# Paleogenomics/pss-bam

Measured on NVIDIA B200. Metric: aligned reads/s (PSS tally), higher is better.
Workload: dtype u64

## Files before the change

### pss-bam_b200/csrc/pss_kernels.cuh

```cuda
#pragma once

#include <cuda_runtime.h>
#include <stdint.h>

#include "pss_record.h"

namespace pssgpu {

__device__ __forceinline__ uint32_t smem_u32(const void *p) { return (uint32_t)__cvta_generic_to_shared(p); }

__device__ __forceinline__ void mbar_init(uint64_t *bar, uint32_t count)
{
    asm volatile("mbarrier.init.shared::cta.b64 [%0], %1;" ::"r"(smem_u32(bar)), "r"(count));
}
__device__ __forceinline__ void fence_mbar_init()
{
    asm volatile("fence.mbarrier_init.release.cluster;" ::: "memory");
}
__device__ __forceinline__ void fence_proxy_async()
{
    asm volatile("fence.proxy.async.shared::cta;" ::: "memory");
}
__device__ __forceinline__ void mbar_expect_tx(uint64_t *bar, uint32_t bytes)
{
// ... 385 lines not shown
        atomicAdd(&s_bins[v.x & 0xffffu], 1u); atomicAdd(&s_bins[v.x >> 16], 1u);
        atomicAdd(&s_bins[v.y & 0xffffu], 1u); atomicAdd(&s_bins[v.y >> 16], 1u);
        atomicAdd(&s_bins[v.z & 0xffffu], 1u); atomicAdd(&s_bins[v.z >> 16], 1u);
        atomicAdd(&s_bins[v.w & 0xffffu], 1u); atomicAdd(&s_bins[v.w >> 16], 1u);
    }
    for (unsigned long long i = a + body * 8 + threadIdx.x; i < hi; i += kSpecSmemThreads) atomicAdd(&s_bins[payload[i]], 1u);
    __syncthreads();
    for (uint32_t i = threadIdx.x; i < (uint32_t)kSpecSmemBins; i += kSpecSmemThreads) {
        const uint32_t v = s_bins[i];
        if (v) atomicAdd(counts + ((size_t)b << kSpecSmemLog) + i, (CT)v);
    }
}
__global__ void __launch_bounds__(256) widen_kernel(const unsigned int *__restrict__ in, unsigned long long *__restrict__ out, uint64_t n)
{
    for (uint64_t i = (uint64_t)blockIdx.x * blockDim.x + threadIdx.x; i < n; i += (uint64_t)gridDim.x * blockDim.x) out[i] = in[i];
}

#ifndef PSS_TALLY_CTAS_PER_SM
#define PSS_TALLY_CTAS_PER_SM 2
#endif
#ifndef PSS_TALLY_THREADS
#define PSS_TALLY_THREADS 256
#endif
#ifndef PSS_TALLY_ITERS
#define PSS_TALLY_ITERS 4
#endif
#ifndef PSS_TALLY_PREFETCH
#define PSS_TALLY_PREFETCH 1
#endif
constexpr int kThreads    = PSS_TALLY_THREADS;
constexpr int kWarps      = kThreads / 32;
#ifndef PSS_TALLY_SLOTS
#define PSS_TALLY_SLOTS (PSS_TALLY_ITERS * PSS_TALLY_THREADS)
#endif
constexpr int kSlots      = PSS_TALLY_SLOTS;
constexpr int kIters      = (kSlots + kThreads - 1) / kThreads;
constexpr int kChunks     = 2 * kSlots;
constexpr int kSpan       = kChunks * 32;
constexpr int kPrefix     = 16;
constexpr int kStageMax   = kSpan - 80;
constexpr int kSegs       = kIters * kWarps;
constexpr int kCacheContigs = 64;
constexpr int kCacheNames   = 1024;
constexpr int kCacheSlots   = 1024;
constexpr int kFlushEvery   = 1900;
static_assert(kThreads % 32 == 0 && kSlots % 32 == 0 && kSegs <= 64, "the newline ranking keeps at most two segment counts per lane");
static_assert(kThreads >= kCacheContigs, "one thread per cached contig fills the shared-memory table");
static_assert(kSpan < (1 << 20) && kThreads <= 1024, "pass A packs a newline position into 20 bits and its rank into the rest");

struct ContigCache {
    uint32_t n;
    uint32_t seed;
    uint16_t name_w0[kCacheContigs], name_len[kCacheContigs];
    uint64_t base_off[kCacheContigs], len[kCacheContigs];
    uint8_t  slot[kCacheSlots];
    uint32_t names32[kCacheNames / 4 + 2 * kCacheContigs];
};

struct TallyShared {
    uint32_t table[2 * 32 * 16];
    uint32_t stats[8];
    uint32_t stats_fk[8];
    ContigCache cc;
};

struct TallySmem {
    alignas(128) uint8_t bytes[kSpan + 32];
    alignas(8) uint32_t le[kChunks + 8];
    uint32_t seg[64];
    uint32_t nlpos[kThreads + 4];
    uint32_t warp_sum[kWarps];
    uint32_t ctl[2];
    unsigned long long long_end;
    TallyShared sh;
    alignas(8) uint64_t bar;
};

struct TallyArgs {
    const uint8_t *sam;
    uint64_t       len;
    const unsigned long long *len_dev;
    uint64_t       stream_off;
    uint64_t       range_bytes;
    unsigned int  *range_ctr;
    uint32_t       one;
    DevGenome      g;
    TallyCfg       cfg;
    TallyCfg       cfg_fk;
    uint32_t       names_bytes;
    uint32_t       cc_seed;
    uint32_t       cc_ok;
    unsigned long long *pss_tables;
    unsigned long long *fk_hist;
    unsigned long long *stats;
    unsigned long long *stats_fk;
    uint64_t           *dbg_off;
    int8_t             *dbg_code;
    unsigned long long *dbg_n;
    uint64_t            dbg_cap;
};

struct SmemAt {
    static constexpr int kLookBack = kPrefix;
    const uint8_t *p;
    __device__ __forceinline__ int lo() const { return 0; }
    __device__ __forceinline__ uint32_t operator()(int i) const { return p[i]; }
    __device__ __forceinline__ uint32_t word(int i) const { return *reinterpret_cast<const uint32_t *>(p + i); }
};
struct SmemRel {
    static constexpr int kLookBack = kPrefix;
    const uint8_t *p;
    __device__ __forceinline__ int lo() const { return -kPrefix; }
    __device__ __forceinline__ uint32_t operator()(int i) const { return p[i]; }
    __device__ __forceinline__ uint32_t word(int i) const
    {
        return (uint32_t)p[i] | ((uint32_t)p[i + 1] << 8) | ((uint32_t)p[i + 2] << 16) | ((uint32_t)p[i + 3] << 24);
    }
};
struct GlobalAt {
    static constexpr int kLookBack = 0;
    const uint8_t *p;
    __device__ __forceinline__ int lo() const { return 0; }
    __device__ __forceinline__ uint32_t operator()(int i) const { return __ldg(p + i); }
    __device__ __forceinline__ uint32_t word(int i) const
    {
        return (uint32_t)__ldg(p + i) | ((uint32_t)__ldg(p + i + 1) << 8) | ((uint32_t)__ldg(p + i + 2) << 16) |
               ((uint32_t)__ldg(p + i + 3) << 24);
    }
};

template <int LUT>
__device__ __forceinline__ uint32_t lop3(uint32_t a, uint32_t b, uint32_t c)
{
    uint32_t d;
    asm("lop3.b32 %0, %1, %2, %3, %4;" : "=r"(d) : "r"(a), "r"(b), "r"(c), "n"(LUT));
    return d;
}
__device__ __forceinline__ uint32_t imad(uint32_t a, uint32_t b, uint32_t c)
{
    uint32_t d;
    asm("mad.lo.u32 %0, %1, %2, %3;" : "=r"(d) : "r"(a), "r"(b), "r"(c));
    return d;
}
__device__ __forceinline__ void classify4(uint32_t w, uint32_t one, uint32_t &zle, uint32_t &znl)
{
    const uint32_t v = w & 0x7f7f7f7fu;
    const uint32_t ge21 = imad(v, one, 0x5f5f5f5fu);
    const uint32_t ge0a = imad(v, one, 0x76767676u);
    const uint32_t ge0b = imad(v, one, 0x75757575u);
    zle = lop3<0x02>(ge21, w, 0x80808080u);
    znl = lop3<0x20>(zle, ge0b, ge0a);
}
__device__ __forceinline__ void classify4_fast(uint32_t w, uint32_t one, uint32_t &zle, uint32_t &p1)
{
    const uint32_t v = w & 0x7f7f7f7fu;
    const uint32_t ge21 = imad(v, one, 0x5f5f5f5fu);
    zle = lop3<0x02>(ge21, w, 0x80808080u);
    p1 = w & 0x02020202u;
}
__device__ __forceinline__ uint32_t gather8(uint32_t z0, uint32_t z1)
{
    return __dp4a(z1, 0x80402010u, __dp4a(z0, 0x08040201u, 0u));
}
__device__ __forceinline__ void classify32(const uint8_t *p, uint32_t one, uint32_t &le32, uint32_t &nl32)
{
    const uint4 v0 = *reinterpret_cast<const uint4 *>(p);
    const uint4 v1 = *reinterpret_cast<const uint4 *>(p + 16);
    uint32_t zl[8], zn[8];
    classify4(v0.x, one, zl[0], zn[0]); classify4(v0.y, one, zl[1], zn[1]);
    classify4(v0.z, one, zl[2], zn[2]); classify4(v0.w, one, zl[3], zn[3]);
    classify4(v1.x, one, zl[4], zn[4]); classify4(v1.y, one, zl[5], zn[5]);
    classify4(v1.z, one, zl[6], zn[6]); classify4(v1.w, one, zl[7], zn[7]);
    le32 = (gather8(zl[0], zl[1]) >> 7) + gather8(zl[2], zl[3]) * 2u + gather8(zl[4], zl[5]) * 512u + gather8(zl[6], zl[7]) * 131072u;
    nl32 = (gather8(zn[0], zn[1]) >> 7) + gather8(zn[2], zn[3]) * 2u + gather8(zn[4], zn[5]) * 512u + gather8(zn[6], zn[7]) * 131072u;
}

__device__ __forceinline__ void classify32_fast(const uint4 &v0, const uint4 &v1, uint32_t one, uint32_t &le32, uint32_t &nc32)
{
    uint32_t zl[8], zp[8];
    classify4_fast(v0.x, one, zl[0], zp[0]); classify4_fast(v0.y, one, zl[1], zp[1]);
    classify4_fast(v0.z, one, zl[2], zp[2]); classify4_fast(v0.w, one, zl[3], zp[3]);
    classify4_fast(v1.x, one, zl[4], zp[4]); classify4_fast(v1.y, one, zl[5], zp[5]);
    classify4_fast(v1.z, one, zl[6], zp[6]); classify4_fast(v1.w, one, zl[7], zp[7]);
    le32 = (gather8(zl[0], zl[1]) >> 7) + gather8(zl[2], zl[3]) * 2u + gather8(zl[4], zl[5]) * 512u + gather8(zl[6], zl[7]) * 131072u;
// ... 372 lines not shown
        r.flag = 0; r.pos = 0; r.mapq = 0; r.tlen = 0;
        r.rname_off = r.cigar_off = r.seq_off = kPrefix; r.rname_len = r.cigar_len = r.seq_len = 0;
    }
    uint64_t   cb, cl;
    const int  ci = lookup_contig(T.cc, A.g, at, r.rname_off, valid ? r.rname_len : 0, cb, cl);
    PssStreams st;
    int        code_fk = code;
    if (MODE != kModePss) {
        FkHits          h;
        const TallyCfg &F = (MODE == kModeBoth) ? A.cfg_fk : A.cfg;
        const int       rc = fk_record(at, r, valid, ci, cb, cl, A.g, F, h);
        if (valid) code_fk = rc;
        if (h.add5) atomicAdd(A.fk_hist + h.idx5, 1ull);
        if (h.add3) atomicAdd(A.fk_hist + (1ull << (2 * F.K)) + h.idx3, 1ull);
    }
    if (MODE != kModeFragkon && NACC == 0) {
        if (valid)
            code = pss_record_wide(at, r, ci, cb, cl, A.g, A.cfg, [&](int tb, int row, int cell) {
                atomicAdd(A.pss_tables + ((size_t)tb * rows + row) * 16 + cell, 1ull);
            });
    } else if (MODE != kModeFragkon) {
        const int rc = pss_record<SmemAt, (ROWS ? ROWS - 2 : -1)>(at, r, valid, ci, cb, cl, A.g, A.cfg, st);
        if (valid) code = rc;
    } else {
        code = code_fk;
    }
    if (code != 99) log_outcome(A, goff, code);
    __syncwarp();
    if (MODE != kModeFragkon && NACC > 0) {
        tally_rows<NACC, ROWS>(st, acc, rows, lane, A.one);
        if (++acc_iters >= kFlushEvery) { flush_acc<NACC>(acc, rows, lane, T.table); acc_iters = 0; }
    }
    {
        const uint32_t m_any = __ballot_sync(full, code != 99);
        const uint32_t m0 = __ballot_sync(full, code == kCounted);
        const uint32_t m1 = __ballot_sync(full, code == kNoContig);
        const uint32_t m2 = __ballot_sync(full, code == kFiltered);
        const uint32_t m3 = __ballot_sync(full, code == kParseFail);
        const uint32_t m4 = __ballot_sync(full, code == kUndefined);
        const uint32_t mine = lane == 0 ? m_any : lane == 1 ? m0 : lane == 2 ? m1 : lane == 3 ? m2 : lane == 4 ? m3 : m4;
        st_acc += (uint32_t)__popc(mine);
        if (MODE == kModeBoth) {
            const uint32_t f0 = __ballot_sync(full, code_fk == kCounted);
            const uint32_t f1 = __ballot_sync(full, code_fk == kNoContig);
            const uint32_t f2 = __ballot_sync(full, code_fk == kFiltered);
            const uint32_t f3 = __ballot_sync(full, code_fk == kParseFail);
            const uint32_t f4 = __ballot_sync(full, code_fk == kUndefined);
            const uint32_t mine_fk = lane == 0 ? m_any : lane == 1 ? f0 : lane == 2 ? f1 : lane == 3 ? f2 : lane == 4 ? f3 : f4;
            st_acc_fk += (uint32_t)__popc(mine_fk);
        }
    }
}

template <int MODE, int NACC, int ROWS>
__global__ void __launch_bounds__(kThreads, PSS_TALLY_CTAS_PER_SM) tally_kernel(const __grid_constant__ TallyArgs A)
{
    extern __shared__ __align__(128) unsigned char smem_raw[];
    TallySmem &S = *reinterpret_cast<TallySmem *>(smem_raw);
    const uint32_t tid = threadIdx.x, lane = tid & 31u, warp = tid >> 5;
    const uint32_t full = 0xffffffffu;
    const uint32_t lt_mask = (1u << lane) - 1u;

    for (uint32_t i = tid; i < 8; i += kThreads) S.le[kChunks + i] = ~0u;
    if (tid < kPrefix) S.bytes[tid] = 'x';
    if (tid == 0) { mbar_init(&S.bar, 1); fence_mbar_init(); }
    cta_prologue(S.sh, A, tid, kThreads);

    const int      rows = A.cfg.R + 2;
    const uint32_t one = A.one;
    uint32_t       phase = 0;
    uint32_t       acc[NACC ? NACC : 1];
    int            acc_iters = 0;
    uint32_t       st_acc = 0, st_acc_fk = 0;
#pragma unroll
    for (int i = 0; i < (NACC ? NACC : 1); i++) acc[i] = 0;
    const uint64_t text_len = A.len_dev ? (uint64_t)__ldg(A.len_dev) : A.len;
    const uint64_t len16 = (text_len + 15) & ~15ull;
    int            est = kStageMax;

    for (;;) {
        __syncthreads();
        if (tid == 0) S.ctl[0] = atomicAdd(A.range_ctr, 1u);
        __syncthreads();
        const uint64_t range_begin = (uint64_t)S.ctl[0] * A.range_bytes;
        if (range_begin >= text_len) break;
        const uint64_t range_end = (range_begin + A.range_bytes < text_len) ? range_begin + A.range_bytes : text_len;
        uint64_t       pos = range_begin;
        bool           want_full = false;

        while (pos < range_end) {
            const uint64_t gsrc = pos ? ((pos - 1) & ~15ull) : 0;
            const int64_t  gbase = (int64_t)gsrc - kPrefix;
            const int      head = (int)((int64_t)pos - 1 - gbase);
            int            want = want_full ? kStageMax : est;
            want = (want + 16) & ~63; want -= 16;
            if (want > kStageMax) want = kStageMax;
            const uint64_t left = len16 - gsrc;
            const bool     sees_end = left <= (uint64_t)want;
            const int      nb = sees_end ? (int)left : want;
            const bool     is_full = sees_end || want >= kStageMax;
            const int      data_end = sees_end ? (int)((int64_t)text_len - gbase) : kPrefix + nb;
            if (tid == 0) {
                fence_proxy_async();
                mbar_expect_tx(&S.bar, (uint32_t)nb);
                bulk_g2s(S.bytes + kPrefix, A.sam + gsrc, (uint32_t)nb, &S.bar);
            }
            if (warp == 0) mbar_wait(&S.bar, phase);
            __syncthreads();
            if (warp != 0) mbar_wait(&S.bar, phase);
            phase ^= 1u;

            const int tail_slot = data_end >> 6;
            const int n_valid = 2 * (sees_end ? tail_slot + 1 : tail_slot);
            if (tid == 0) {
                S.bytes[kPrefix - 1] = pos == 0 ? '\n' : 'x';
                for (int i = kPrefix; i < head; i++) S.bytes[i] = 'x';
            }
            if (sees_end && tid == (uint32_t)(tail_slot % kThreads)) {
                S.bytes[data_end] = '\n';
                for (int i = data_end + 1; i < 64 * (tail_slot + 1); i++) S.bytes[i] = 'x';
            }

            constexpr uint32_t kNoNl = 0xfffffu;
            uint32_t pk[kIters];
            uint32_t redo = 0;
            const uint32_t r4 = (lane >> 1) & 3u;
            const uint32_t qo0 = 16u * r4, qo1 = 16u * (1u ^ r4), qo2 = 16u * (2u ^ r4), qo3 = 16u * (3u ^ r4);
            const uint32_t rot16 = 16u * (r4 & 1u), hi_x = r4 >> 1, swz = 16u * r4;
#pragma unroll
            for (int it = 0; it < kIters; it++) {
                pk[it] = kNoNl;
                if (it * 2 * kThreads < n_valid + 8 && ((it + 1) * kThreads <= kSlots || it * kThreads + (int)tid < kSlots)) {
                    const int      c = 2 * (it * kThreads + (int)tid);
                    const uint8_t *src = S.bytes + 32 * c;
                    const uint4    q0 = *reinterpret_cast<const uint4 *>(src + qo0), q1 = *reinterpret_cast<const uint4 *>(src + qo1);
                    const uint4    q2 = *reinterpret_cast<const uint4 *>(src + qo2), q3 = *reinterpret_cast<const uint4 *>(src + qo3);
                    uint32_t le_x, nc_x, le_y, nc_y;
                    classify32_fast(q0, q1, one, le_x, nc_x);
                    classify32_fast(q2, q3, one, le_y, nc_y);
                    le_x = __funnelshift_l(le_x, le_x, rot16);
                    le_y = __funnelshift_l(le_y, le_y, rot16);
                    S.le[c + (int)hi_x] = le_x;
                    S.le[c + 1 - (int)hi_x] = le_y;
                    const bool     has = (nc_x | nc_y) != 0u && c < n_valid;
                    const uint32_t b = __ballot_sync(full, has);
                    const uint32_t rank = (uint32_t)__popc(b & lt_mask);
                    const uint32_t x = nc_x ? nc_x : nc_y;
                    const uint32_t p = (uint32_t)(32 * c) + ((((nc_x ? 0u : 32u) + (uint32_t)__ffs((int)x) - 1u) ^ swz) & 63u);
                    redo |= has ? ((x & (x - 1u)) | (nc_x ? nc_y : 0u) | ((uint32_t)S.bytes[has ? p : 0u] ^ 0x0au)) : 0u;
                    pk[it] = has ? (p + (rank << 20)) : kNoNl;
                    if (lane == 0) S.seg[it * kWarps + (int)warp] = b;
                } else if (lane == 0) {
                    S.seg[it * kWarps + (int)warp] = 0u;
                }
            }
            const int any_multi = __syncthreads_or((int)(redo != 0u));
            if (tid < 8) S.le[n_valid + (int)tid] = ~0u;

            uint32_t n_nl;
            if (!any_multi) {
                uint32_t v0 = (lane < (uint32_t)kSegs) ? (uint32_t)__popc(S.seg[lane]) : 0u;
                uint32_t v1 = (kSegs > 32 && lane + 32 < (uint32_t)kSegs) ? (uint32_t)__popc(S.seg[lane + 32]) : 0u;
                uint32_t x = v0 | (v1 << 16);
                uint32_t inc = x;
#pragma unroll
                for (int d = 1; d < 32; d <<= 1) {
                    const uint32_t t = __shfl_up_sync(full, inc, d);
                    if ((int)lane >= d) inc += t;
                }
// ... 74 lines not shown
#endif
constexpr int kWSlots    = PSS_WTILE_SLOTS;
constexpr int kWIters    = (kWSlots + 31) / 32;
constexpr int kWChunks   = 2 * kWSlots;
constexpr int kWSpan     = kWChunks * 32;
constexpr int kWStageMax = kWSpan - 80;
static_assert(kWSlots % 32 == 0, "whole warp steps");

struct WarpTile {
    alignas(128) uint8_t bytes[kWSpan + 32];
    alignas(8) uint32_t le[kWChunks + 8];
    uint32_t nlpos[36];
    alignas(8) uint64_t bar;
};
struct TallyWarpSmem {
    WarpTile    w[kWarps];
    TallyShared sh;
};

__device__ __noinline__ uint32_t wlist_newlines_generic(WarpTile *Wp, int n_valid, uint32_t one)
{
    WarpTile      &W = *Wp;
    const uint32_t lane = threadIdx.x & 31u, full = 0xffffffffu;
    const int      per = (n_valid + 31) / 32, c0 = (int)lane * per;
    uint32_t       sum = 0;
    for (int k = 0; k < per; k++) {
        if (c0 + k >= n_valid) break;
        uint32_t le32, nl32;
        classify32(W.bytes + 32 * (c0 + k), one, le32, nl32);
        sum += (uint32_t)__popc(nl32);
    }
    uint32_t inc = sum;
#pragma unroll
    for (int d = 1; d < 32; d <<= 1) {
        const uint32_t t = __shfl_up_sync(full, inc, d);
        if ((int)lane >= d) inc += t;
    }
    const uint32_t total = __shfl_sync(full, inc, 31);
    uint32_t ord = inc - sum;
    for (int k = 0; k < per; k++) {
        if (c0 + k >= n_valid) break;
        uint32_t le32, nl32;
        classify32(W.bytes + 32 * (c0 + k), one, le32, nl32);
        while (nl32) {
            if (ord <= 32u) W.nlpos[ord] = (uint32_t)((c0 + k) * 32 + __ffs((int)nl32) - 1);
            nl32 &= nl32 - 1u;
            ord++;
        }
    }
    return total;
}

template <int MODE, int NACC, int ROWS>
__global__ void __launch_bounds__(kThreads, PSS_TALLY_CTAS_PER_SM) tally_warp_kernel(const __grid_constant__ TallyArgs A)
{
    extern __shared__ __align__(128) unsigned char smem_raw[];
    TallyWarpSmem &S = *reinterpret_cast<TallyWarpSmem *>(smem_raw);
    const uint32_t tid = threadIdx.x, lane = tid & 31u, warp = tid >> 5;
    const uint32_t full = 0xffffffffu;
    const uint32_t lt_mask = (1u << lane) - 1u;
    WarpTile      &W = S.w[warp];

    if (lane < 8) W.le[kWChunks + lane] = ~0u;
    if (lane < kPrefix) W.bytes[lane] = 'x';
    if (lane == 0) { mbar_init(&W.bar, 1); fence_mbar_init(); }
    cta_prologue(S.sh, A, tid, kThreads);

    const int      rows = A.cfg.R + 2;
    const uint32_t one = A.one;
    uint32_t       phase = 0;
    uint32_t       acc[NACC ? NACC : 1];
    int            acc_iters = 0;
    uint32_t       st_acc = 0, st_acc_fk = 0;
#pragma unroll
    for (int i = 0; i < (NACC ? NACC : 1); i++) acc[i] = 0;
    const uint64_t text_len = A.len_dev ? (uint64_t)__ldg(A.len_dev) : A.len;
    const uint64_t len16 = (text_len + 15) & ~15ull;
    int            est = kWStageMax;

    for (;;) {
        uint32_t r = 0;
        if (lane == 0) r = atomicAdd(A.range_ctr, 1u);
        r = __shfl_sync(full, r, 0);
        const uint64_t range_begin = (uint64_t)r * A.range_bytes;
        if (range_begin >= text_len) break;
        const uint64_t range_end = (range_begin + A.range_bytes < text_len) ? range_begin + A.range_bytes : text_len;
        uint64_t       pos = range_begin;
        bool           want_full = false;

        while (pos < range_end) {
            const uint64_t gsrc = pos ? ((pos - 1) & ~15ull) : 0;
            const int64_t  gbase = (int64_t)gsrc - kPrefix;
            const int      head = (int)((int64_t)pos - 1 - gbase);
            int            want = want_full ? kWStageMax : est;
            want = (want + 16) & ~63; want -= 16;
            if (want > kWStageMax) want = kWStageMax;
            const uint64_t left = len16 - gsrc;
            const bool     sees_end = left <= (uint64_t)want;
            const int      nb = sees_end ? (int)left : want;
            const bool     is_full = sees_end || want >= kWStageMax;
            const int      data_end = sees_end ? (int)((int64_t)text_len - gbase) : kPrefix + nb;
            __syncwarp();
            if (lane == 0) {
                fence_proxy_async();
                mbar_expect_tx(&W.bar, (uint32_t)nb);
                bulk_g2s(W.bytes + kPrefix, A.sam + gsrc, (uint32_t)nb, &W.bar);
            }
            mbar_wait(&W.bar, phase);
            phase ^= 1u;

            const int tail_slot = data_end >> 6;
            const int n_valid = 2 * (sees_end ? tail_slot + 1 : tail_slot);
            if (lane == 0) {
                W.bytes[kPrefix - 1] = pos == 0 ? '\n' : 'x';
                for (int i = kPrefix; i < head; i++) W.bytes[i] = 'x';
            }
            if (sees_end && lane == (uint32_t)(tail_slot & 31)) {
                W.bytes[data_end] = '\n';
                for (int i = data_end + 1; i < 64 * (tail_slot + 1); i++) W.bytes[i] = 'x';
            }
            __syncwarp();

            constexpr uint32_t kNoNl = 0xfffffu;
            uint32_t pk[kWIters], bal[kWIters];
            uint32_t redo = 0;
            const uint32_t r4 = (lane >> 1) & 3u;
            const uint32_t qo0 = 16u * r4, qo1 = 16u * (1u ^ r4), qo2 = 16u * (2u ^ r4), qo3 = 16u * (3u ^ r4);
            const uint32_t rot16 = 16u * (r4 & 1u), hi_x = r4 >> 1, swz = 16u * r4;
#pragma unroll
            for (int it = 0; it < kWIters; it++) {
                pk[it] = kNoNl;
                bal[it] = 0u;
                if (it * 64 < n_valid + 8) {
                    const int      c = 2 * (it * 32 + (int)lane);
                    const uint8_t *src = W.bytes + 32 * c;
                    const uint4    q0 = *reinterpret_cast<const uint4 *>(src + qo0), q1 = *reinterpret_cast<const uint4 *>(src + qo1);
                    const uint4    q2 = *reinterpret_cast<const uint4 *>(src + qo2), q3 = *reinterpret_cast<const uint4 *>(src + qo3);
                    uint32_t le_x, nc_x, le_y, nc_y;
                    classify32_fast(q0, q1, one, le_x, nc_x);
                    classify32_fast(q2, q3, one, le_y, nc_y);
                    le_x = __funnelshift_l(le_x, le_x, rot16);
                    le_y = __funnelshift_l(le_y, le_y, rot16);
                    W.le[c + (int)hi_x] = le_x;
                    W.le[c + 1 - (int)hi_x] = le_y;
                    const bool     has = (nc_x | nc_y) != 0u && c < n_valid;
                    const uint32_t b = __ballot_sync(full, has);
                    const uint32_t rank = (uint32_t)__popc(b & lt_mask);
                    const uint32_t x = nc_x ? nc_x : nc_y;
                    const uint32_t p = (uint32_t)(32 * c) + ((((nc_x ? 0u : 32u) + (uint32_t)__ffs((int)x) - 1u) ^ swz) & 63u);
                    redo |= has ? ((x & (x - 1u)) | (nc_x ? nc_y : 0u) | ((uint32_t)W.bytes[has ? p : 0u] ^ 0x0au)) : 0u;
                    pk[it] = has ? (p + (rank << 20)) : kNoNl;
                    bal[it] = b;
                }
            }
            const bool any_multi = __any_sync(full, redo != 0u);
            __syncwarp();
            if (lane < 8) W.le[n_valid + (int)lane] = ~0u;

            uint32_t n_nl;
            if (!any_multi) {
                uint32_t base = 0;
#pragma unroll
                for (int it = 0; it < kWIters; it++) {
                    const uint32_t v = pk[it];
                    const uint32_t ord = base + (v >> 20);
                    if (v != kNoNl && ord <= 32u) W.nlpos[ord] = v & 0xfffffu;
                    base += (uint32_t)__popc(bal[it]);
                }
                n_nl = base;
// ... 64 lines not shown
```

### pss-bam_b200/csrc/pss_record.h

```cpp
#pragma once

#include <stdint.h>

#if defined(__CUDACC__)
#define PSS_HD __host__ __device__ __forceinline__
#define PSS_HD_NOINLINE __host__ __device__ __noinline__
#else
#define PSS_HD inline
#define PSS_HD_NOINLINE inline
#endif

namespace pssgpu {

constexpr int      kBasesPerGroup = 16;
constexpr int      kPadGroups     = 4;
constexpr int      kPadBases      = kPadGroups * kBasesPerGroup;
constexpr uint32_t kSymOther      = 15;

struct DevContig {
    uint64_t base_off;
    uint64_t len;
    uint32_t name_off;
    uint32_t name_len;
};
// ... 165 lines not shown
            if (!is_ws(c)) break;
            i++;
        }
        if (c == 0) return kParseFail;
        const bool is_str = (conv == 0 || conv == 2 || conv == 5 || conv == 6 || conv == 9 || conv == 10);
        if (is_str) {
            int st = i;
            while (i < L) { c = b(i); if (c == 0 || is_ws(c)) break; i++; }
            int len = i - st;
            if (conv == 2)  { r.rname_off = st; r.rname_len = len; }
            if (conv == 5)  { r.cigar_off = st; r.cigar_len = len; }
            if (conv == 9)  { r.seq_off = st;   r.seq_len = len; }
            if (conv == 10) qual_len = len;
        } else {
            bool neg = false;
            if (c == '+' || c == '-') { neg = (c == '-'); i++; c = i < L ? b(i) : 0u; }
            uint32_t base = 10;
            int      nd = 0;
            uint64_t v = 0;
            bool     ovf = false;
            if (conv == 8 && c == '0') {
                uint32_t c1 = (i + 1 < L) ? b(i + 1) : 0u;
                if ((c1 | 32u) == 'x') { base = 16; i += 2; nd = 1; }
                else base = 8;
            }
            for (;;) {
                c = i < L ? b(i) : 0u;
                uint32_t d;
                if (is_digit(c)) d = c - '0';
                else if (base == 16 && (((c | 32u) - 'a') <= 5u)) d = (c | 32u) - 'a' + 10;
                else break;
                if (d >= base) break;
                if (v > (~0ull - d) / base) ovf = true; else v = v * base + d;
                nd++;
                i++;
            }
            if (nd == 0) return kParseFail;
            if (conv == 8) {
                int64_t x;
                if (!neg) x = (ovf || v > 0x7fffffffffffffffull) ? 0x7fffffffffffffffll : (int64_t)v;
                else      x = (ovf || v > 0x8000000000000000ull) ? (int64_t)0x8000000000000000ull : (int64_t)(0ull - v);
                r.tlen = (int32_t)(uint32_t)(uint64_t)x;
            } else {
                const uint64_t x = ovf ? ~0ull : (neg ? 0ull - v : v);
                if (conv == 1) r.flag = (uint32_t)x;
                if (conv == 3) r.pos = x;
                if (conv == 4) r.mapq = (uint32_t)x;
            }
        }
    }
    if (r.seq_len != qual_len) return kParseFail;
    return kCounted;
}

template <class B>
PSS_HD uint32_t word_at(const B &b, int p)
{
    const int a = p & ~3;
    return funnel_r(b.word(a), b.word(a + 4), 8u * (uint32_t)(p & 3));
}
PSS_HD bool all_digits4(uint32_t t) { return (((t + 0x76767676u) | t) & 0x80808080u) == 0u; }
PSS_HD uint32_t value4(uint32_t t)
{
    t = t * 10u + (t >> 8);
    return (t & 0xffu) * 100u + ((t >> 16) & 0xffu);
}
PSS_HD uint32_t digit_tail(uint32_t w, int drop)
{
#if defined(__CUDA_ARCH__)
    const uint32_t m = __funnelshift_lc(0u, 0xffffffffu, 8u * (uint32_t)drop);
#else
    const uint32_t m = drop >= 4 ? 0u : (0xffffffffu << (8 * drop));
#endif
    return (w ^ 0x30303030u) & m;
}
template <class B>
PSS_HD uint32_t dec_loop(const B &b, int a, int e, bool &ok)
{
    uint32_t v = 0;
    for (int i = a; i < e; i++) { const uint32_t d = b(i) - '0'; ok = ok && (d <= 9u); v = v * 10u + d; }
    return v;
}
template <class B>
PSS_HD uint32_t dec4(const B &b, int a, int e, bool &ok)
{
    int L = e - a;
    ok = ok && (L >= 1) && (L <= 4);
    if (!ok) L = 1;
    if (B::kLookBack < 4 && e - 4 < b.lo()) return dec_loop(b, e - L, e, ok);
    const uint32_t t = digit_tail(word_at(b, e - 4), 4 - L);
    ok = ok && all_digits4(t);
    return value4(t);
}
template <class B>
PSS_HD void digits9(const B &b, int a, int e, bool &ok)
{
    int L = e - a;
    ok = ok && (L >= 1) && (L <= 9);
    if (!ok) L = 1;
    if (B::kLookBack < 12 && e - 12 < b.lo()) { (void)dec_loop(b, e - L, e, ok); return; }
    const int      p = e - 12, a0 = p & ~3, drop = 12 - L;
    const uint32_t sh = 8u * (uint32_t)(p & 3);
    const uint32_t x0 = b.word(a0), x1 = b.word(a0 + 4), x2 = b.word(a0 + 8), x3 = b.word(a0 + 12);
    const uint32_t t0 = digit_tail(funnel_r(x0, x1, sh), drop);
    const uint32_t t1 = digit_tail(funnel_r(x1, x2, sh), drop - 4 < 0 ? 0 : drop - 4);
    const uint32_t t2 = digit_tail(funnel_r(x2, x3, sh), drop - 8 < 0 ? 0 : drop - 8);
    ok = ok && all_digits4(t0) && all_digits4(t1) && all_digits4(t2);
}
template <class B>
PSS_HD uint32_t dec9(const B &b, int a, int e, bool &ok)
{
    int L = e - a;
    ok = ok && (L >= 1) && (L <= 9);
    if (!ok) L = 1;
    if (B::kLookBack < 12 && e - 12 < b.lo()) return dec_loop(b, e - L, e, ok);
    const int      p = e - 12, a0 = p & ~3, drop = 12 - L;
    const uint32_t sh = 8u * (uint32_t)(p & 3);
    const uint32_t x0 = b.word(a0), x1 = b.word(a0 + 4), x2 = b.word(a0 + 8), x3 = b.word(a0 + 12);
    const uint32_t t0 = digit_tail(funnel_r(x0, x1, sh), drop);
    const uint32_t t1 = digit_tail(funnel_r(x1, x2, sh), drop - 4 < 0 ? 0 : drop - 4);
    const uint32_t t2 = digit_tail(funnel_r(x2, x3, sh), drop - 8 < 0 ? 0 : drop - 8);
    ok = ok && all_digits4(t0) && all_digits4(t1) && all_digits4(t2);
    return (value4(t0) * 10000u + value4(t1)) * 10000u + value4(t2);
}

template <class B>
PSS_HD int split_fast(const B &b, const uint32_t *le, int p0, int pe, RecView &r)
{
    int      sep[11];
    int      w = p0 >> 5;
    uint32_t bits = le[w] & (0xffffffffu << (p0 & 31));
    int      prev = p0 - 1;
    bool     ok = true;
#define PSS_NEXT_SEP(f)                                                                         \
    do {                                                                                        \
        while (bits == 0) {                                                                     \
            const uint32_t b1 = le[w + 1], b2 = le[w + 2], b3 = le[w + 3], b4 = le[w + 4];      \
            const int      k = b1 ? 1 : b2 ? 2 : b3 ? 3 : 4;                                    \
            bits = b1 ? b1 : b2 ? b2 : b3 ? b3 : b4;                                            \
            w += k;                                                                             \
        }                                                                                       \
        int p = (w << 5) + ffs32(bits) - 1;                                                     \
        bits &= bits - 1;                                                                       \
        if (p > pe) p = pe;                                                                     \
        ok = ok && (p > prev + 1);                    \
        if ((f) < 10) ok = ok && (p < pe);          \
        sep[f] = p;                                                                             \
        prev = p;                                                                               \
    } while (0)
    {
        const uint32_t b1 = le[w + 1], b2 = le[w + 2];
        const bool     h0 = bits != 0u, h1 = b1 != 0u;
        const uint32_t x = h0 ? bits : h1 ? b1 : b2;
        w += h0 ? 0 : h1 ? 1 : 2;
        bits = x;
    }
    PSS_NEXT_SEP(0);
    {
        int            cur = sep[0] + 1;
        const int      w0 = cur >> 5;
        const uint32_t s0 = (uint32_t)(cur & 31);
        const uint32_t q0 = le[w0], q1 = le[w0 + 1], q2 = le[w0 + 2], q3 = le[w0 + 3];
        uint32_t h0 = funnel_r(q0, q1, s0), h1 = funnel_r(q1, q2, s0), h2 = funnel_r(q2, q3, s0);
#pragma unroll
        for (int f = 1; f <= 8; f++) {
            const int t = ffs32(h0);
            ok = ok && (t > 1);
            cur += t;
            sep[f] = cur - 1;
#if !defined(__CUDA_ARCH__)
            if (sep[f] > pe) sep[f] = pe;
#endif
            h0 = funnel_rc(h0, h1, (uint32_t)t);
            h1 = funnel_rc(h1, h2, (uint32_t)t);
            h2 = funnel_rc(h2, 0u, (uint32_t)t);
        }
        ok = ok && (sep[8] < pe);
        prev = sep[8];
        w = cur >> 5;
        bits = le[w] & (0xffffffffu << (cur & 31));
    }
#define PSS_SKIP5()                                                                             \
    do {                                                                                        \
        const uint32_t b1 = le[w + 1], b2 = le[w + 2], b3 = le[w + 3], b4 = le[w + 4], b5 = le[w + 5]; \
        const bool     h0 = bits != 0u, h1 = b1 != 0u, h2 = b2 != 0u, h3 = b3 != 0u, h4 = b4 != 0u;    \
        const uint32_t x = h0 ? bits : h1 ? b1 : h2 ? b2 : h3 ? b3 : h4 ? b4 : b5;              \
        w += h0 ? 0 : h1 ? 1 : h2 ? 2 : h3 ? 3 : h4 ? 4 : 5;                                    \
        bits = x;                                                                               \
    } while (0)
    PSS_SKIP5();
    PSS_NEXT_SEP(9);
    PSS_SKIP5();
    PSS_NEXT_SEP(10);
#undef PSS_SKIP5
#undef PSS_NEXT_SEP
#pragma unroll
    for (int f = 0; f < 10; f++) ok = ok && (b(sep[f]) == '\t');
    ok = ok && (sep[10] == pe || is_ws(b(sep[10])));

    const int qname_len = sep[0] - p0;
    r.rname_off = sep[1] + 1; r.rname_len = sep[2] - sep[1] - 1;
    r.cigar_off = sep[4] + 1; r.cigar_len = sep[5] - sep[4] - 1;
    const int mrnm_len = sep[6] - sep[5] - 1;
    r.seq_off = sep[8] + 1;   r.seq_len = sep[9] - sep[8] - 1;
    const int qual_len = sep[10] - sep[9] - 1;
    ok = ok && ((qname_len | r.rname_len | r.cigar_len | mrnm_len | r.seq_len | qual_len) <= kMaxField);

    r.flag = dec4(b, sep[0] + 1, sep[1], ok);
    r.pos = dec9(b, sep[2] + 1, sep[3], ok);
    r.mapq = dec4(b, sep[3] + 1, sep[4], ok);
    digits9(b, sep[6] + 1, sep[7], ok);
    {
        int a = sep[7] + 1;
        const int e = sep[8];
        const uint32_t c = b(a);
        const bool neg = (c == '-');
        if (c == '-' || c == '+') a++;
        ok = ok && !(e - a > 1 && b(a) == '0');
        const uint32_t v = dec4(b, a, e, ok);
        r.tlen = neg ? -(int32_t)v : (int32_t)v;
    }
    if (!ok) return kNeedSlow;
    if (r.seq_len != qual_len) return kParseFail;
    return kCounted;
}

template <class B>
PSS_HD int find_contig(const DevGenome &g, const B &b, int off, int len)
{
    uint32_t h = kNameHashSeed;
    for (int i = 0; i < len; i++) h = name_hash_step(h, (uint8_t)b(off + i));
    uint32_t slot = h & g.hash_mask;
    for (;;) {
        uint32_t v = g.hash[slot];
        if (v == 0) return -1;
        const DevContig &c = g.contigs[v - 1];
        if ((int)c.name_len == len) {
            const char *nm = g.names + c.name_off;
            int i = 0;
            while (i < len && (uint8_t)nm[i] == (uint8_t)b(off + i)) i++;
            if (i == len) return (int)(v - 1);
        }
        slot = (slot + 1) & g.hash_mask;
    }
}

struct RawWindow {
    uint64_t g0, g1, g2;
    uint32_t sh;
};
PSS_HD RawWindow fetch_window(const DevGenome &g, uint64_t gb, int n_fields)
{
    RawWindow w;
    const uint64_t gi = gb >> 4;
    const uint32_t o = (uint32_t)(gb & 15u);
    w.sh = 2 * o;
    w.g0 = g.groups[gi];
    w.g1 = g.groups[gi + 1];
    w.g2 = (o + (uint32_t)n_fields > 32u) ? g.groups[gi + 2] : 0ull;
    return w;
}
PSS_HD void window_fields(const RawWindow &w, int n_fields, uint32_t late, uint64_t &codes, uint64_t &classes)
{
    const uint32_t sh = w.sh | late;
    const uint32_t c_lo = funnel_r((uint32_t)w.g0, (uint32_t)w.g1, sh);
    const uint32_t c_hi = funnel_r((uint32_t)w.g1, (uint32_t)w.g2, sh);
    const uint32_t k_lo = funnel_r((uint32_t)(w.g0 >> 32), (uint32_t)(w.g1 >> 32), sh);
    const uint32_t k_hi = funnel_r((uint32_t)(w.g1 >> 32), (uint32_t)(w.g2 >> 32), sh);
    const uint64_t m = low_fields_mask(n_fields);
    codes   = (((uint64_t)c_hi << 32) | c_lo) & m;
    classes = (((uint64_t)k_hi << 32) | k_lo) & m;
}
PSS_HD void load_window(const DevGenome &g, uint64_t gb, int n_fields, uint64_t &codes, uint64_t &classes)
{
    window_fields(fetch_window(g, gb, n_fields), n_fields, 0u, codes, classes);
}

PSS_HD uint8_t other_char(const DevGenome &g, uint64_t gb)
{
    uint32_t lo = 0, hi = g.n_exc;
    while (lo < hi) {
        uint32_t mid = lo + (hi - lo) / 2;
        uint64_t p = g.exc_pos[mid];
        if (p == gb) return g.exc_chr[mid];
        if (p < gb) lo = mid + 1; else hi = mid;
    }
    return 0xff;
}

PSS_HD bool ctx_member(const DevGenome &g, const TallyCfg &P, bool down, uint32_t sym, bool complement, uint64_t gb, bool live)
{
    if (sym < 4u && complement) sym ^= 3u;
    const uint32_t mask = down ? P.down_mask : P.up_mask;
    if (sym != kSymOther || !live) return ((mask >> (sym & 15u)) & 1u) != 0u;
    if (!(down ? P.down_other : P.up_other)) return false;
    const uint8_t c = other_char(g, gb);
    const char *s = down ? P.down_ctx : P.up_ctx;
    for (int i = 0; i < kMaxCtxChars && s[i]; i++)
        if ((uint8_t)s[i] == c) return true;
    return false;
}

template <class B>
PSS_HD bool cigar_is_nM(const B &b, int off, int len, int64_t n)
{
    bool ok = (len >= 2) && (len <= 10) && (n >= 0);
    if (!ok) len = 2;
    ok = ok && (b(off + len - 1) == 'M') && !(b(off) == '0' && len != 2);
    if (n >= 10000) {
        const uint32_t v = dec9(b, off, off + len - 1, ok);
        return ok && (int64_t)v == n;
    }
    ok = ok && (len <= 5);
    if (!ok) len = 2;
    const uint32_t v = dec4(b, off, off + len - 1, ok);
    return ok && (int64_t)v == n;
}

PSS_HD uint32_t byte_perm(uint32_t x, uint32_t y, uint32_t sel)
{
#if defined(__CUDA_ARCH__)
    return __byte_perm(x, y, sel);
#else
    const uint64_t src = ((uint64_t)y << 32) | x;
    uint32_t out = 0;
    for (int i = 0; i < 4; i++) out |= (uint32_t)((src >> (8 * ((sel >> (4 * i)) & 7u))) & 0xffu) << (8 * i);
    return out;
#endif
}
PSS_HD void codes_of_word(uint32_t w, uint32_t &codes8, uint32_t &bad8)
{
    const uint32_t c = w | 0x20202020u;
    const uint32_t k = (c >> 1) & 0x03030303u;
    uint32_t sel = (k | (k >> 4)) & 0x00330033u;
    sel = (sel | (sel >> 8)) & 0x3333u;
    const uint32_t x = c ^ byte_perm(0x67746361u, 0u, sel);
    const uint32_t nz = (((x & 0x7f7f7f7fu) + 0x7f7f7f7fu) | x) & 0x80808080u;
    const uint32_t code = k ^ ((k >> 1) & 0x01010101u);
    codes8 = (code * 0x01041040u) >> 24;
    bad8 = ((nz >> 7) * 0x01041040u) >> 24;
}
template <class B, int NWC = 0>
PSS_HD void read_codes(const B &b, int off, int n_words, uint64_t &codes, uint64_t &bad)
{
    if (NWC) n_words = NWC;
    codes = 0; bad = 0;
    const int      a0 = off & ~3;
    const uint32_t sh = 8u * (uint32_t)(off & 3);
    uint32_t       prev = b.word(a0);
#pragma unroll
    for (int k = 0; k < 8; k++) {
        if (k >= n_words) break;
        const uint32_t next = b.word(a0 + 4 * k + 4);
        uint32_t c8, b8;
        codes_of_word(funnel_r(prev, next, sh), c8, b8);
        codes |= (uint64_t)c8 << (8 * k);
        bad   |= (uint64_t)b8 << (8 * k);
        prev = next;
    }
}

struct PssStreams {
    uint64_t a_ref, a_read, a_bad;
    uint64_t b_ref, b_read, b_bad;
};

constexpr uint64_t kEvenBits = 0x5555555555555555ull;

template <class B, int RC = -1>
PSS_HD int pss_record(const B &b, const RecView &r, bool valid, int ci, uint64_t ctg_base, uint64_t ctg_len,
                      const DevGenome &g, const TallyCfg &P, PssStreams &st)
{
    int  code = kCounted;
    bool live = valid;
#define PSS_DROP(cond, c) do { if (live && (cond)) { code = (c); live = false; } } while (0)
    PSS_DROP(ci < 0, kNoContig);
    PSS_DROP(ctg_len == 0, kUndefined);

    const bool paired = r.flag & 1u;
    const uint32_t abs_tlen = r.tlen < 0 ? 0u - (uint32_t)r.tlen : (uint32_t)r.tlen;
    const int64_t  n = (int64_t)(paired ? abs_tlen : (uint32_t)r.seq_len);
    PSS_DROP(n > kMaxTlen, kUndefined);
    const int     R = RC >= 0 ? RC : P.R;
    const int64_t s = (int64_t)(r.pos - 1);
    const int64_t e = s + n - 1;

    PSS_DROP(s - 2 < 0, kFiltered);
    PSS_DROP((uint64_t)(e + 2) > ctg_len - 1, kFiltered);
    PSS_DROP(r.mapq < P.min_mq, kFiltered);
    PSS_DROP(!((uint64_t)n >= P.min_len && (uint64_t)n <= P.max_len && n >= R), kFiltered);
    PSS_DROP(r.flag & (4u | 256u | 512u | 1024u | 2048u), kFiltered);
    PSS_DROP(P.merged_only && paired, kFiltered);

    const int W = R + 2;
    uint64_t lc, lk, rc, rk;
    const RawWindow lw = fetch_window(g, live ? ctg_base + (uint64_t)(s - 2) : (uint64_t)kPadBases, W);
    const RawWindow rw = fetch_window(g, live ? ctg_base + (uint64_t)(e + 2 - (W - 1)) : (uint64_t)kPadBases, W);

// ... 174 lines not shown
```

### pss-bam_b200/csrc/pssgpu.cu

```cuda
#include "pssgpu_internal.h"

#include <unistd.h>

#include <algorithm>
#include <cstdlib>
#include <cstring>

#include "pss_kernels.cuh"

using namespace pssgpu;

namespace {
constexpr bool   kTallyWarpDefault = false;
constexpr size_t kPackPiece   = 128ull << 20;
constexpr uint64_t kExcCap    = 4ull << 20;
thread_local std::string g_init_error;
}

namespace pssgpu {

int fail(pssgpu_ctx *c, int code, const char *fmt, ...)
{
    char buf[512];
    va_list ap;
// ... 196 lines not shown
        return fail(ctx, PSSGPU_EUNSUPP, "genome_upload: a contig contains a NUL byte");
    }
    if (exc_n > kExcCap) {
        ctx->exc_overflow = true;
        ctx->n_exc = 0;
    } else if (exc_n > 0) {
        std::vector<uint64_t> pos(exc_n);
        std::vector<uint8_t>  chr(exc_n);
        CUX(cudaMemcpy(pos.data(), ctx->d_exc_pos, exc_n * sizeof(uint64_t), cudaMemcpyDeviceToHost));
        CUX(cudaMemcpy(chr.data(), ctx->d_exc_chr, exc_n, cudaMemcpyDeviceToHost));
        std::vector<uint32_t> order(exc_n);
        for (uint32_t k = 0; k < exc_n; k++) order[k] = k;
        std::sort(order.begin(), order.end(), [&](uint32_t a, uint32_t b) { return pos[a] < pos[b]; });
        std::vector<uint64_t> spos(exc_n);
        std::vector<uint8_t>  schr(exc_n);
        for (uint32_t k = 0; k < exc_n; k++) { spos[k] = pos[order[k]]; schr[k] = chr[order[k]]; }
        CUX(cudaMemcpy(ctx->d_exc_pos, spos.data(), exc_n * sizeof(uint64_t), cudaMemcpyHostToDevice));
        CUX(cudaMemcpy(ctx->d_exc_chr, schr.data(), exc_n, cudaMemcpyHostToDevice));
        ctx->n_exc = (uint32_t)exc_n;
    }
    CUX(cudaMalloc(&ctx->d_contigs, std::max<size_t>(1, n) * sizeof(DevContig)));
    CUX(cudaMalloc(&ctx->d_names, names.size() + 16));
    CUX(cudaMalloc(&ctx->d_hash, hash_size * sizeof(uint32_t)));
    if (n) CUX(cudaMemcpy(ctx->d_contigs, tab.data(), n * sizeof(DevContig), cudaMemcpyHostToDevice));
    if (!names.empty()) CUX(cudaMemcpy(ctx->d_names, names.data(), names.size(), cudaMemcpyHostToDevice));
    CUX(cudaMemcpy(ctx->d_hash, hash.data(), hash_size * sizeof(uint32_t), cudaMemcpyHostToDevice));
    cleanup();
#undef CUX
    ctx->hash_mask = hash_size - 1;
    ctx->names_bytes = (uint32_t)names.size();
    ctx->cc_seed = cc_seed;
    ctx->cc_ok = cc_ok;
    ctx->n_groups = n_groups;
    ctx->n_bases = total;
    ctx->n_contigs = n;
    ctx->genome_bytes = n_groups * sizeof(uint64_t) + kExcCap * 9 + n * sizeof(DevContig) + names.size() + hash_size * 4;
    ctx->have_genome = true;
    return PSSGPU_OK;
}

int ctx_string(pssgpu_ctx *ctx, const char *s, uint32_t *mask, uint32_t *other, char *copy)
{
    static const char named[] = PSSGPU_SYM_CHARS;
    *mask = 0; *other = 0;
    memset(copy, 0, kMaxCtxChars);
    if (!s) return fail(ctx, PSSGPU_EINVAL, "context string is null");
    const size_t n = strlen(s);
    if (n >= (size_t)kMaxCtxChars) return fail(ctx, PSSGPU_EUNSUPP, "context string longer than %d bytes", kMaxCtxChars - 1);
    memcpy(copy, s, n);
    for (size_t i = 0; i < n; i++) {
        const char *p = strchr(named, s[i]);
        if (p && *p) *mask |= 1u << (p - named);
        else *other = 1;
    }
    return PSSGPU_OK;
}

template <int MODE>
int launch_tally(pssgpu_ctx *ctx, const uint8_t *d_sam, size_t len, uint64_t stream_off, const unsigned long long *len_dev)
{
    if (len == 0) return PSSGPU_OK;
    TallyArgs a;
    a.sam = d_sam; a.len = len; a.stream_off = stream_off;
    a.len_dev = len_dev;
    a.g = dev_genome(ctx);
    a.cfg = ctx->cfg;
    a.cfg_fk = ctx->cfg_fk;
    a.names_bytes = ctx->names_bytes;
    a.cc_seed = ctx->cc_seed;
    a.cc_ok = ctx->cc_ok;
    a.pss_tables = ctx->d_tables;
    a.fk_hist = ctx->d_fk;
    a.stats = ctx->d_stats;
    a.stats_fk = ctx->d_stats + kStN;
    a.dbg_off = ctx->dbg ? ctx->d_dbg_off : nullptr;
    a.dbg_code = ctx->dbg ? ctx->d_dbg_code : nullptr;
    a.dbg_n = ctx->dbg ? ctx->d_dbg_n : nullptr;
    a.dbg_cap = ctx->dbg_cap;
    const int      max_grid = MODE == kModeFragkon ? ctx->tally_grid_fk : ctx->tally_grid_pss;
    uint64_t rb = len / ((uint64_t)max_grid * (ctx->tally_warp ? 8u * (uint64_t)kWarps : 8u));
    if (const char *e = getenv("PSSGPU_RANGE_KB")) rb = std::max<uint64_t>(1, strtoull(e, nullptr, 10)) << 10;
    else rb = std::min<uint64_t>(std::max<uint64_t>(rb, ctx->tally_warp ? (32u << 10) : (128u << 10)), 1u << 20);
    rb = (rb + 31) & ~31ull;
    const uint64_t n_ranges = (len + rb - 1) / rb;
    a.range_bytes = rb;
    a.range_ctr = ctx->d_range_ctr;
    a.one = 1u;
    CU(cudaMemsetAsync(ctx->d_range_ctr, 0, sizeof(unsigned int), ctx->stream));
    time_begin(ctx, len);
    const unsigned grid = (unsigned)std::min<uint64_t>(ctx->tally_warp ? (n_ranges + kWarps - 1) / kWarps : n_ranges, (uint64_t)max_grid);
    constexpr int PM = MODE == kModeFragkon ? kModePss : MODE;
#define PSS_LAUNCH(KERNEL, SMEM)                                                                                          \
    do {                                                                                                                 \
        if (MODE == kModeFragkon) KERNEL<kModeFragkon, 9, 0><<<grid, kThreads, SMEM, ctx->stream>>>(a);                  \
        else if (ctx->cfg.R == 15) KERNEL<PM, 9, 17><<<grid, kThreads, SMEM, ctx->stream>>>(a);        \
        else if (ctx->cfg.R + 2 <= 18) KERNEL<PM, 9, 0><<<grid, kThreads, SMEM, ctx->stream>>>(a);                       \
        else if (ctx->cfg.R <= kMaxRegion) KERNEL<PM, 16, 0><<<grid, kThreads, SMEM, ctx->stream>>>(a);                  \
        else KERNEL<PM, 0, 0><<<grid, kThreads, SMEM, ctx->stream>>>(a);                   \
    } while (0)
    if (ctx->tally_warp) PSS_LAUNCH(tally_warp_kernel, sizeof(TallyWarpSmem));
    else PSS_LAUNCH(tally_kernel, sizeof(TallySmem));
#undef PSS_LAUNCH
    time_end(ctx);
    CU(cudaGetLastError());
    return PSSGPU_OK;
}

}

int pssgpu::launch_tally_mode(pssgpu_ctx *ctx, const uint8_t *d_sam, size_t len, uint64_t stream_off, const unsigned long long *len_dev)
{
    return ctx->mode == kModePss  ? launch_tally<kModePss>(ctx, d_sam, len, stream_off, len_dev)
         : ctx->mode == kModeBoth ? launch_tally<kModeBoth>(ctx, d_sam, len, stream_off, len_dev)
                                  : launch_tally<kModeFragkon>(ctx, d_sam, len, stream_off, len_dev);
}

namespace {

int begin_common(pssgpu_ctx *ctx)
{
    CU(cudaStreamSynchronize(ctx->stream));
    if (!ctx->d_stats) CU(cudaMalloc(&ctx->d_stats, 2 * kStN * sizeof(unsigned long long)));
    if (!ctx->d_range_ctr) CU(cudaMalloc(&ctx->d_range_ctr, sizeof(unsigned int)));
    CU(cudaMemsetAsync(ctx->d_stats, 0, 2 * kStN * sizeof(unsigned long long), ctx->stream));
    if (ctx->d_dbg_n) CU(cudaMemsetAsync(ctx->d_dbg_n, 0, sizeof(unsigned long long), ctx->stream));
    ctx->carry_len = 0;
    ctx->cur = 0;
    ctx->fed_bytes = 0;
    bam_reset(ctx);
    return PSSGPU_OK;
}

}

extern "C" {

int pssgpu_abi_version(void) { return PSSGPU_ABI_VERSION; }

int pssgpu_device_count(void)
{
    int n = 0;
    if (cudaGetDeviceCount(&n) != cudaSuccess) { cudaGetLastError(); return -1; }
    return n;
}

int pssgpu_init(int device, pssgpu_ctx **out)
{
    pssgpu_ctx *ctx = nullptr;
    if (!out) return fail(nullptr, PSSGPU_EINVAL, "pssgpu_init: out is null");
    *out = nullptr;
    int n = 0;
    CU(cudaGetDeviceCount(&n));
    if (device < 0 || device >= n) return fail(nullptr, PSSGPU_EINVAL, "pssgpu_init: device %d of %d", device, n);
    cudaDeviceProp prop;
    CU(cudaGetDeviceProperties(&prop, device));
    if (prop.major != 10)
        return fail(nullptr, PSSGPU_EUNSUPP, "pssgpu_init: device %d is sm_%d%d; this library holds sm_100a code only",
                    device, prop.major, prop.minor);
    CU(cudaSetDevice(device));
    pssgpu_ctx *c = new pssgpu_ctx();
    c->device = device;
    c->sm_count = prop.multiProcessorCount;
    cudaError_t e = cudaStreamCreateWithFlags(&c->stream, cudaStreamNonBlocking);
    if (e == cudaSuccess) e = cudaEventCreateWithFlags(&c->copy_done, cudaEventDisableTiming);
    if (e == cudaSuccess) e = cudaStreamCreateWithFlags(&c->copy_stream, cudaStreamNonBlocking);
    for (int i = 0; i < 2; i++) {
        if (e == cudaSuccess) e = cudaEventCreateWithFlags(&c->ev_copied[i], cudaEventDisableTiming);
        if (e == cudaSuccess) e = cudaEventCreateWithFlags(&c->ev_tallied[i], cudaEventDisableTiming);
// ... 761 lines not shown
```

Baseline: 9.139 billion.

## Use smaller tail ranges for load balance and fold delimiter checks into number decoding

Work ranges are now split into large ranges followed by smaller tail ranges of about one-eighth size, so the last wave of CTAs finishes more evenly and tail imbalance shrinks. Separately, the SAM field decoders (dec4/dec9/digits9) now also return the byte after each number from the already-loaded words. This replaces five of the ten separator tab checks, and dec9 reuses a shared digits12 helper with a combined validity test. The change adds some index arithmetic per range claim and rearranges the parser's validation logic.

```diff
diff --git a/pss-bam_b200/csrc/pss_kernels.cuh b/pss-bam_b200/csrc/pss_kernels.cuh
--- a/pss-bam_b200/csrc/pss_kernels.cuh
+++ b/pss-bam_b200/csrc/pss_kernels.cuh
@@ -491,6 +491,8 @@
     const unsigned long long *len_dev;
     uint64_t       stream_off;
     uint64_t       range_bytes;
+    uint64_t       tail_bytes;
+    uint32_t       n_big;
     unsigned int  *range_ctr;
     uint32_t       one;
     DevGenome      g;
@@ -509,6 +511,13 @@
     uint64_t            dbg_cap;
 };
 
+__device__ __forceinline__ void range_of(const TallyArgs &A, uint32_t c, uint64_t text_len, uint64_t &begin, uint64_t &end)
+{
+    const bool     big = c < A.n_big;
+    const uint64_t n = big ? A.range_bytes : A.tail_bytes;
+    begin = big ? (uint64_t)c * A.range_bytes : (uint64_t)A.n_big * A.range_bytes + (uint64_t)(c - A.n_big) * A.tail_bytes;
+    end = begin + n < text_len ? begin + n : text_len;
+}
 struct SmemAt {
     static constexpr int kLookBack = kPrefix;
     const uint8_t *p;
@@ -1047,9 +1056,9 @@
         __syncthreads();
         if (tid == 0) S.ctl[0] = atomicAdd(A.range_ctr, 1u);
         __syncthreads();
-        const uint64_t range_begin = (uint64_t)S.ctl[0] * A.range_bytes;
+        uint64_t range_begin, range_end;
+        range_of(A, S.ctl[0], text_len, range_begin, range_end);
         if (range_begin >= text_len) break;
-        const uint64_t range_end = (range_begin + A.range_bytes < text_len) ? range_begin + A.range_bytes : text_len;
         uint64_t       pos = range_begin;
         bool           want_full = false;
 
@@ -1290,9 +1299,9 @@
         uint32_t r = 0;
         if (lane == 0) r = atomicAdd(A.range_ctr, 1u);
         r = __shfl_sync(full, r, 0);
-        const uint64_t range_begin = (uint64_t)r * A.range_bytes;
+        uint64_t range_begin, range_end;
+        range_of(A, r, text_len, range_begin, range_end);
         if (range_begin >= text_len) break;
-        const uint64_t range_end = (range_begin + A.range_bytes < text_len) ? range_begin + A.range_bytes : text_len;
         uint64_t       pos = range_begin;
         bool           want_full = false;
 
diff --git a/pss-bam_b200/csrc/pss_record.h b/pss-bam_b200/csrc/pss_record.h
--- a/pss-bam_b200/csrc/pss_record.h
+++ b/pss-bam_b200/csrc/pss_record.h
@@ -271,46 +271,54 @@
     return v;
 }
 template <class B>
-PSS_HD uint32_t dec4(const B &b, int a, int e, bool &ok)
+PSS_HD uint32_t dec4(const B &b, int a, int e, bool &ok, uint32_t &after)
 {
     int L = e - a;
     ok = ok && (L >= 1) && (L <= 4);
     if (!ok) L = 1;
-    if (B::kLookBack < 4 && e - 4 < b.lo()) return dec_loop(b, e - L, e, ok);
-    const uint32_t t = digit_tail(word_at(b, e - 4), 4 - L);
+    if (B::kLookBack < 4 && e - 4 < b.lo()) { after = b(e); return dec_loop(b, e - L, e, ok); }
+    const int      a0 = (e - 4) & ~3;
+    const uint32_t sh = 8u * (uint32_t)(e & 3);
+    const uint32_t x0 = b.word(a0), x1 = b.word(a0 + 4);
+    after = (x1 >> sh) & 0xffu;
+    const uint32_t t = digit_tail(funnel_r(x0, x1, sh), 4 - L);
     ok = ok && all_digits4(t);
     return value4(t);
 }
 template <class B>
-PSS_HD void digits9(const B &b, int a, int e, bool &ok)
+PSS_HD bool digits12(const B &b, int e, int L, uint32_t &t0, uint32_t &t1, uint32_t &t2, uint32_t &after)
+{
+    const int      p = e - 12, a0 = p & ~3, drop = 12 - L;
+    const uint32_t sh = 8u * (uint32_t)(p & 3);
+    const uint32_t x0 = b.word(a0), x1 = b.word(a0 + 4), x2 = b.word(a0 + 8), x3 = b.word(a0 + 12);
+    after = (x3 >> sh) & 0xffu;
+    t0 = digit_tail(funnel_r(x0, x1, sh), drop);
+    t1 = digit_tail(funnel_r(x1, x2, sh), drop - 4 < 0 ? 0 : drop - 4);
+    t2 = digit_tail(funnel_r(x2, x3, sh), drop - 8 < 0 ? 0 : drop - 8);
+    return ((((t0 + 0x76767676u) | t0) | ((t1 + 0x76767676u) | t1) | ((t2 + 0x76767676u) | t2)) & 0x80808080u) == 0u;
+}
+template <class B>
+PSS_HD void digits9(const B &b, int a, int e, bool &ok, uint32_t &after)
 {
     int L = e - a;
     ok = ok && (L >= 1) && (L <= 9);
     if (!ok) L = 1;
-    if (B::kLookBack < 12 && e - 12 < b.lo()) { (void)dec_loop(b, e - L, e, ok); return; }
-    const int      p = e - 12, a0 = p & ~3, drop = 12 - L;
-    const uint32_t sh = 8u * (uint32_t)(p & 3);
-    const uint32_t x0 = b.word(a0), x1 = b.word(a0 + 4), x2 = b.word(a0 + 8), x3 = b.word(a0 + 12);
-    const uint32_t t0 = digit_tail(funnel_r(x0, x1, sh), drop);
-    const uint32_t t1 = digit_tail(funnel_r(x1, x2, sh), drop - 4 < 0 ? 0 : drop - 4);
-    const uint32_t t2 = digit_tail(funnel_r(x2, x3, sh), drop - 8 < 0 ? 0 : drop - 8);
-    ok = ok && all_digits4(t0) && all_digits4(t1) && all_digits4(t2);
-}
-template <class B>
-PSS_HD uint32_t dec9(const B &b, int a, int e, bool &ok)
+    if (B::kLookBack < 12 && e - 12 < b.lo()) { after = b(e); (void)dec_loop(b, e - L, e, ok); return; }
+    uint32_t   t0, t1, t2;
+    const bool digits = digits12(b, e, L, t0, t1, t2, after);
+    ok = ok && digits;
+}
+template <class B>
+PSS_HD uint32_t dec9(const B &b, int a, int e, bool &ok, uint32_t &after)
 {
     int L = e - a;
     ok = ok && (L >= 1) && (L <= 9);
     if (!ok) L = 1;
-    if (B::kLookBack < 12 && e - 12 < b.lo()) return dec_loop(b, e - L, e, ok);
-    const int      p = e - 12, a0 = p & ~3, drop = 12 - L;
-    const uint32_t sh = 8u * (uint32_t)(p & 3);
-    const uint32_t x0 = b.word(a0), x1 = b.word(a0 + 4), x2 = b.word(a0 + 8), x3 = b.word(a0 + 12);
-    const uint32_t t0 = digit_tail(funnel_r(x0, x1, sh), drop);
-    const uint32_t t1 = digit_tail(funnel_r(x1, x2, sh), drop - 4 < 0 ? 0 : drop - 4);
-    const uint32_t t2 = digit_tail(funnel_r(x2, x3, sh), drop - 8 < 0 ? 0 : drop - 8);
-    ok = ok && all_digits4(t0) && all_digits4(t1) && all_digits4(t2);
-    return (value4(t0) * 10000u + value4(t1)) * 10000u + value4(t2);
+    if (B::kLookBack < 12 && e - 12 < b.lo()) { after = b(e); return dec_loop(b, e - L, e, ok); }
+    uint32_t   t0, t1, t2;
+    const bool digits = digits12(b, e, L, t0, t1, t2, after);
+    ok = ok && digits;
+    return ((t0 >> 24) * 10000u + value4(t1)) * 10000u + value4(t2);
 }
 
 template <class B>
@@ -383,8 +391,7 @@
     PSS_NEXT_SEP(10);
 #undef PSS_SKIP5
 #undef PSS_NEXT_SEP
-#pragma unroll
-    for (int f = 0; f < 10; f++) ok = ok && (b(sep[f]) == '\t');
+    ok = ok && (b(sep[0]) == '\t') && (b(sep[2]) == '\t') && (b(sep[5]) == '\t') && (b(sep[6]) == '\t') && (b(sep[9]) == '\t');
     ok = ok && (sep[10] == pe || is_ws(b(sep[10])));
 
     const int qname_len = sep[0] - p0;
@@ -395,10 +402,15 @@
     const int qual_len = sep[10] - sep[9] - 1;
     ok = ok && ((qname_len | r.rname_len | r.cigar_len | mrnm_len | r.seq_len | qual_len) <= kMaxField);
 
-    r.flag = dec4(b, sep[0] + 1, sep[1], ok);
-    r.pos = dec9(b, sep[2] + 1, sep[3], ok);
-    r.mapq = dec4(b, sep[3] + 1, sep[4], ok);
-    digits9(b, sep[6] + 1, sep[7], ok);
+    uint32_t after;
+    r.flag = dec4(b, sep[0] + 1, sep[1], ok, after);
+    ok = ok && after == '\t';
+    r.pos = dec9(b, sep[2] + 1, sep[3], ok, after);
+    ok = ok && after == '\t';
+    r.mapq = dec4(b, sep[3] + 1, sep[4], ok, after);
+    ok = ok && after == '\t';
+    digits9(b, sep[6] + 1, sep[7], ok, after);
+    ok = ok && after == '\t';
     {
         int a = sep[7] + 1;
         const int e = sep[8];
@@ -406,7 +418,8 @@
         const bool neg = (c == '-');
         if (c == '-' || c == '+') a++;
         ok = ok && !(e - a > 1 && b(a) == '0');
-        const uint32_t v = dec4(b, a, e, ok);
+        const uint32_t v = dec4(b, a, e, ok, after);
+        ok = ok && after == '\t';
         r.tlen = neg ? -(int32_t)v : (int32_t)v;
     }
     if (!ok) return kNeedSlow;
@@ -497,12 +510,14 @@
     if (!ok) len = 2;
     ok = ok && (b(off + len - 1) == 'M') && !(b(off) == '0' && len != 2);
     if (n >= 10000) {
-        const uint32_t v = dec9(b, off, off + len - 1, ok);
+        uint32_t       after;
+        const uint32_t v = dec9(b, off, off + len - 1, ok, after);
         return ok && (int64_t)v == n;
     }
     ok = ok && (len <= 5);
     if (!ok) len = 2;
-    const uint32_t v = dec4(b, off, off + len - 1, ok);
+    uint32_t       after;
+    const uint32_t v = dec4(b, off, off + len - 1, ok, after);
     return ok && (int64_t)v == n;
 }
 
diff --git a/pss-bam_b200/csrc/pssgpu.cu b/pss-bam_b200/csrc/pssgpu.cu
--- a/pss-bam_b200/csrc/pssgpu.cu
+++ b/pss-bam_b200/csrc/pssgpu.cu
@@ -302,8 +302,17 @@
     if (const char *e = getenv("PSSGPU_RANGE_KB")) rb = std::max<uint64_t>(1, strtoull(e, nullptr, 10)) << 10;
     else rb = std::min<uint64_t>(std::max<uint64_t>(rb, ctx->tally_warp ? (32u << 10) : (128u << 10)), 1u << 20);
     rb = (rb + 31) & ~31ull;
-    const uint64_t n_ranges = (len + rb - 1) / rb;
+    uint64_t       rb_tail = rb, n_big = (len + rb - 1) / rb;
+    const uint64_t tail = (uint64_t)max_grid * rb;
+    if (!getenv("PSSGPU_RANGE_KB") && !ctx->tally_warp && len > 4 * tail) {
+        rb_tail = std::max<uint64_t>(rb / 8, 64u << 10);
+        rb_tail = (rb_tail + 31) & ~31ull;
+        n_big = (len - tail) / rb;
+    }
+    const uint64_t n_ranges = n_big + (len - std::min(len, n_big * rb) + rb_tail - 1) / rb_tail;
     a.range_bytes = rb;
+    a.tail_bytes = rb_tail;
+    a.n_big = (uint32_t)n_big;
     a.range_ctr = ctx->d_range_ctr;
     a.one = 1u;
     CU(cudaMemsetAsync(ctx->d_range_ctr, 0, sizeof(unsigned int), ctx->stream));
```

Result: faster. 9.269 billion (median of 6 runs) (+1.4%).
